# gabrielfnayres/new-vit

Hardware: AMD Instinct MI355X
Metric: volumes_per_sec_mst_dinov2_fwd (higher is better)
Workload: dtype bf16; 1 GPU; MST-DINOv2 (DinoV2ClassifierSlice, ViT-S/14) forward, 4 volumes/GPU of 64x512x512 bf16 zero-padded to 518x518 (N=1370 tokens/slice); global_batch_volumes=4, slices=64, parallelism=single GPU, weights=synthetic (mst.synth seed 2), random init of the reference architecture

## Files before the change

### new-vit_amd/csrc/k_attn16.hip

```cpp
#include <type_traits>

#include "mst_common.h"

namespace {

constexpr float LOG2E = 1.4426950408889634f;
constexpr int KV_TILE_BYTES = 64 * 128;
constexpr int K_ROW = 144, K_TILE_BYTES = 64 * K_ROW;

template <typename T>
__device__ __forceinline__ typename V8<T>::type tr_pair(const char* p_lo, const char* p_hi) {
    typedef typename V8<T>::type vec8;
    union { struct { s16x4 lo, hi; } s; vec8 v; } u;
    u.s.lo = __builtin_amdgcn_ds_read_tr16_b64_v4i16((__attribute__((address_space(3))) s16x4*)(p_lo));
    u.s.hi = __builtin_amdgcn_ds_read_tr16_b64_v4i16((__attribute__((address_space(3))) s16x4*)(p_hi));
    return u.v;
}

constexpr int ATTN_WG_WAVES = 4;
constexpr int WGW = ATTN_WG_WAVES, WGT = 64 * WGW, QB = 32 * WGW;
constexpr int ATTN_WAVES_PER_EU = 4;
template <typename T>
__global__ __launch_bounds__(WGT) __attribute__((amdgpu_waves_per_eu(ATTN_WAVES_PER_EU, ATTN_WAVES_PER_EU))) void attn16_kernel(const T* __restrict__ qkv, T* __restrict__ out,
                                                     int N, int heads, int log2q, int out_blocked) {
    typedef typename V8<T>::type vec8;
    __shared__ __attribute__((aligned(16))) char smem[4 * KV_TILE_BYTES];
    char* const Ks = smem;
    char* const Vs = smem + 2 * KV_TILE_BYTES;

    const int tid = threadIdx.x, lane = tid & 63;
    const int wave = __builtin_amdgcn_readfirstlane(tid >> 6);
    const int nqb = (N + QB - 1) / QB;
    const int tile = xcd_remap(blockIdx.x, gridDim.x);
    const int qb = tile % nqb, h = (tile / nqb) % heads, seq = tile / (nqb * heads);
    const int E = heads * 64, ld = 3 * E;
    const T* base = qkv + (int64_t)seq * N * ld;
    const int h2 = lane >> 5;

    const int q = qb * QB + wave * 32 + (lane & 31);
    const bool wave_active = (qb * QB + wave * 32) < N;
    vec8 bq[4];
    {
        const int qc = q < N ? q : N - 1;
        const T* qp = base + (int64_t)qc * ld + h * 64 + h2 * 8;
#pragma unroll
        for (int ds = 0; ds < 4; ++ds) bq[ds] = *reinterpret_cast<const vec8*>(qp + ds * 16);
    }

    static_assert(WGW == 4 || WGW == 8, "the LDS-DMA staging map deals 16 pieces per tile to 4 or 8 waves");
    constexpr int PPW = 16 / WGW;
    const int d_p0 = wave * PPW;
    const int d_row0 = (d_p0 & 7) * 8 + (lane >> 3);
    const int d_isv = d_p0 >> 3;
    const int d_chunk0 = d_isv ? ((lane & 7) ^ (((d_row0 >> 1) & 1) << 2)) : ((lane & 7) ^ ((d_row0 >> 1) & 7));
    const int d_col0 = (1 + d_isv) * (heads * 64) + h * 64 + d_chunk0 * 8;
    unsigned d_off[PPW];
#pragma unroll
    for (int u = 0; u < PPW; ++u) d_off[u] = (unsigned)(((d_row0 + 8 * u) * ld + ((u & 1) && !d_isv ? (d_col0 ^ 32) : d_col0)) * 2);
    auto dma = [&](int t, int buf) {
        char* dst = (d_isv ? Vs + buf * KV_TILE_BYTES : Ks + buf * KV_TILE_BYTES) + (d_p0 & 7) * 1024;
        if (t * 64 + 64 <= N) {
            const char* tb = reinterpret_cast<const char*>(base) + (int64_t)t * 64 * ld * 2;
#pragma unroll
            for (int u = 0; u < PPW; ++u) {
                const unsigned m0v = (unsigned)(size_t)(__attribute__((address_space(3))) char*)(dst + u * 1024);
#pragma clang diagnostic push
#pragma clang diagnostic ignored "-Winline-asm"
                asm volatile("s_mov_b32 m0, %2\n\ts_nop 0\n\tglobal_load_lds_dwordx4 %0, %1"
                             :
                             : "v"(d_off[u]), "s"(tb), "s"(m0v)
                             : "memory", "m0");
#pragma clang diagnostic pop
            }
        } else {
#pragma unroll
            for (int u = 0; u < PPW; ++u) {
                int key = t * 64 + d_row0 + 8 * u;
                key = key < N ? key : N - 1;
                const int col = (u & 1) && !d_isv ? (d_col0 ^ 32) : d_col0;
                __builtin_amdgcn_global_load_lds(GLB_PTR(base + (int64_t)key * ld + col), LDS_PTR(dst + u * 1024), 16, 0, 0);
            }
        }
    };
    const int krow = lane & 31;
    int k_off4[4];
#pragma unroll
    for (int ds = 0; ds < 4; ++ds) k_off4[ds] = krow * 128 + (((2 * ds + h2) ^ ((krow >> 1) & 7)) << 4);
    const int vi = lane & 15;
    const int vrow = 4 * h2 + (vi >> 2);
    const int vsw = ((vrow >> 1) & 1) << 2;
    const int vchunk = ((lane >> 4) & 1) * 2 + ((vi & 3) >> 1);
    const int v_lane_off = vrow * 128 + (vi & 1) * 8;

    f32x16 oT[2];
#pragma unroll
    for (int r = 0; r < 16; ++r) oT[0][r] = oT[1][r] = 0.f;
    if (!log2q) {
#pragma unroll
        for (int ds = 0; ds < 4; ++ds)
#pragma unroll
            for (int j = 0; j < 8; ++j) bq[ds][j] = (T)((float)bq[ds][j] * LOG2E);
    }
    float r_ref = 0.f, l_run = 0.f;
    constexpr float RT = 8.0f;

    const int nt = (N + 63) >> 6;
    dma(0, 0);
    asm volatile("s_waitcnt vmcnt(0)" ::: "memory");
    __syncthreads();

    constexpr float TH0 = std::is_same<T, f16_t>::value ? 8.0f : 60.0f;
    constexpr float GUARD = std::is_same<T, f16_t>::value ? 32768.0f : 1.2676506e30f;
    bool fast = false;

    auto tile_step = [&](auto mask_tag, auto fast_tag, int t, bool skip_dma) -> bool {
        constexpr bool MASK = decltype(mask_tag)::value;
        constexpr bool FAST = decltype(fast_tag)::value;
        const int buf = t & 1;
        if (t + 1 < nt && !skip_dma) dma(t + 1, buf ^ 1);
        if (wave_active) {
            const char* Kb = Ks + buf * KV_TILE_BYTES;
            const char* Vb = Vs + buf * KV_TILE_BYTES;
            f32x16 s[2];
            const f32x16 zero16 = {0.f, 0.f, 0.f, 0.f, 0.f, 0.f, 0.f, 0.f, 0.f, 0.f, 0.f, 0.f, 0.f, 0.f, 0.f, 0.f};
            const bool upper = !MASK || (t * 64 + 32 < N);
            auto scores = [&](bool with_ref) {
                vec8 kone, qneg;
                if (with_ref) {
#pragma unroll
                    for (int j = 0; j < 8; ++j) kone[j] = qneg[j] = (T)0.f;
                    if (h2 == 0) {
                        kone[0] = (T)1.f;
                        qneg[0] = (T)(-r_ref);
                    }
                }
#pragma unroll
                for (int kb = 0; kb < 2; ++kb) {
                    if (MASK && kb == 1 && !upper) {
#pragma unroll
                        for (int r = 0; r < 16; ++r) s[1][r] = -INFINITY;
                        continue;
                    }
                    s[kb] = with_ref ? mfma32(kone, qneg, zero16) : zero16;
#pragma unroll
                    for (int ds = 0; ds < 4; ++ds) {
                        const vec8 a = *reinterpret_cast<const vec8*>(Kb + k_off4[ds] + kb * 4096);
                        s[kb] = mfma32(a, bq[ds], s[kb]);
                    }
                }
                if constexpr (MASK) {
#pragma unroll
                    for (int kb = 0; kb < 2; ++kb)
#pragma unroll
                        for (int r = 0; r < 16; ++r) {
                            const int key = t * 64 + kb * 32 + (r & 3) + 8 * (r >> 2) + 4 * h2;
                            if (key >= N) s[kb][r] = -INFINITY;
                        }
                }
            };
            float lsum;
            vec8 pf[4];
            auto exps = [&]() {
                lsum = 0.f;
#pragma unroll
                for (int kb = 0; kb < 2; ++kb)
#pragma unroll
                    for (int r = 0; r < 16; ++r) {
                        const float p = __builtin_amdgcn_exp2f(s[kb][r]);
                        s[kb][r] = p;
                        lsum += p;
                    }
#pragma unroll
                for (int ks = 0; ks < 4; ++ks)
#pragma unroll
                    for (int j = 0; j < 8; ++j) pf[ks][j] = (T)s[ks >> 1][(ks & 1) * 8 + j];
            };
            auto classic = [&]() {
                float mx = s[0][0];
#pragma unroll
                for (int r = 1; r < 16; ++r) mx = fmaxf(mx, s[0][r]);
#pragma unroll
                for (int r = 0; r < 16; ++r) mx = fmaxf(mx, s[1][r]);
                {
                    const unsigned mu = __float_as_uint(mx);
                    const auto sw = __builtin_amdgcn_permlane32_swap(mu, mu, false, false);
                    mx = fmaxf(__uint_as_float(sw[0]), __uint_as_float(sw[1]));
                }
                if (t == 0 && __all(fabsf(mx) <= TH0)) {
                    fast = true;
                } else if (t == 0 || !__all(mx <= RT)) {
                    const bool mv = (t == 0) || (mx > RT);
                    const float r_new = mv ? (float)(T)(r_ref + mx) : r_ref;
                    const float delta = r_new - r_ref;
                    const float alpha = t == 0 ? 1.0f : __builtin_amdgcn_exp2f(-delta);
                    r_ref = r_new;
                    l_run *= alpha;
#pragma unroll
                    for (int r = 0; r < 16; ++r) {
                        oT[0][r] *= alpha;
                        oT[1][r] *= alpha;
                        s[0][r] -= delta;
                        s[1][r] -= delta;
                    }
                }
                exps();
            };
            if constexpr (FAST) {
                scores(false);
                exps();
                if (!__all(lsum < GUARD)) return false;
            } else {
                scores(true);
                classic();
            }
            l_run += lsum;
#pragma unroll
            for (int ks = 0; ks < 4; ++ks) {
                if (MASK && ks >= 2 && !upper) continue;
#pragma unroll
                for (int db = 0; db < 2; ++db) {
                    const char* p = Vb + ks * 16 * 128 + v_lane_off + (((db * 4 + vchunk) ^ vsw) * 16);
                    const vec8 vf = tr_pair<T>(p, p + 8 * 128);
                    oT[db] = mfma32(vf, pf[ks], oT[db]);
                }
            }
        }
        asm volatile("s_waitcnt vmcnt(0)" ::: "memory");
        __syncthreads();
        return true;
    };
    const int nt_full = (N & 63) ? nt - 1 : nt;
    const std::false_type FULL{}, CLASSIC{};
    const std::true_type RAGGED{}, FASTM{};
    if (nt_full > 0) tile_step(FULL, CLASSIC, 0, false);
    else tile_step(RAGGED, CLASSIC, 0, false);
    int t = 1;
    bool resume = false;
    if (fast) {
        for (; t < nt_full; ++t)
            if (!tile_step(FULL, FASTM, t, false)) { resume = true; break; }
    }
    for (; t < nt_full; ++t) {
        tile_step(FULL, CLASSIC, t, resume);
        resume = false;
    }
    if (t < nt) tile_step(RAGGED, CLASSIC, t, resume);

    if (wave_active) {
        const float l_tot = l_run + __shfl_xor(l_run, 32, 64);
        const float inv = 1.0f / l_tot;
        if (q < N) {
            const int64_t R = (int64_t)seq * N + q;
            T* op = out_blocked ? out + (R >> 5) * (32 * E) + (4 * h) * 512 + (R & 31) * 8 + 4 * h2
                                : out + R * E + h * 64 + 4 * h2;
            const int sdb = out_blocked ? 1024 : 32, sg2 = out_blocked ? 512 : 16, sg1 = out_blocked ? 256 : 8;
#pragma unroll
            for (int db = 0; db < 2; ++db)
#pragma unroll
                for (int g = 0; g < 4; ++g) {
                    typedef __attribute__((ext_vector_type(4))) T o4;
                    o4 pk;
#pragma unroll
                    for (int e = 0; e < 4; ++e) pk[e] = (T)(oT[db][g * 4 + e] * inv);
                    *reinterpret_cast<o4*>(op + db * sdb + (g >> 1) * sg2 + (g & 1) * sg1) = pk;
                }
        }
    }
}

template <typename T>
__global__ __launch_bounds__(256) void cls_probs_kernel(const T* __restrict__ qkv, float* __restrict__ probs,
                                                        int N, int heads, int hd, int log2q, T* __restrict__ attn_out = nullptr) {
    extern __shared__ float sm[];
    float* q0 = sm;
    float* sc = sm + hd;
    float* red = sc + N;
    const int h = blockIdx.x, seq = blockIdx.y, tid = threadIdx.x;
    const int E = heads * hd, ld = 3 * E;
    const T* base = qkv + (int64_t)seq * N * ld;
    for (int d = tid; d < hd; d += 256) q0[d] = to_f32(base[h * hd + d]);
    __syncthreads();
    float mx = -INFINITY;
    if (hd == 64) {
        const int sub = tid & 7;
        float qr[8];
#pragma unroll
        for (int i = 0; i < 8; ++i) qr[i] = q0[sub * 8 + i];
        for (int j0 = 0; j0 < N; j0 += 32) {
            const int j = j0 + (tid >> 3);
            const T* kp = base + (int64_t)(j < N ? j : N - 1) * ld + E + h * 64 + sub * 8;
            float a = 0.f;
#pragma unroll
            for (int i = 0; i < 8; ++i) a = fmaf(qr[i], to_f32(kp[i]), a);
            a += __shfl_xor(a, 1, 64);
            a += __shfl_xor(a, 2, 64);
            a += __shfl_xor(a, 4, 64);
            if (j < N) {
                if (sub == 0) sc[j] = a;
                mx = fmaxf(mx, a);
            }
        }
    } else {
        for (int j = tid; j < N; j += 256) {
            const T* kp = base + (int64_t)j * ld + E + h * hd;
            float a = 0.f;
            for (int d = 0; d < hd; ++d) a = fmaf(q0[d], to_f32(kp[d]), a);
            sc[j] = a;
            mx = fmaxf(mx, a);
        }
    }
    mx = wave_max(mx);
    if ((tid & 63) == 0) red[tid >> 6] = mx;
    __syncthreads();
    mx = fmaxf(fmaxf(red[0], red[1]), fmaxf(red[2], red[3]));
    float sum = 0.f;
    for (int j = tid; j < N; j += 256) {
        const float p = log2q ? exp2f(sc[j] - mx) : __expf(sc[j] - mx);
        sc[j] = p;
        sum += p;
    }
    sum = wave_sum(sum);
    if ((tid & 63) == 0) red[4 + (tid >> 6)] = sum;
    __syncthreads();
    const float inv = 1.0f / (red[4] + red[5] + red[6] + red[7]);
    if (probs) {
        float* po = probs + ((int64_t)seq * heads + h) * N;
        for (int j = tid; j < N; j += 256) po[j] = sc[j] * inv;
    }
    if (attn_out) {
        float* part = red + 8;
        const int d = tid & 63, pt = tid >> 6;
        const int per = (N + 3) >> 2;
        const int j1 = (pt + 1) * per < N ? (pt + 1) * per : N;
        float a = 0.f;
        for (int j = pt * per; j < j1; ++j) a = fmaf(sc[j], to_f32(base[(int64_t)j * ld + 2 * E + h * 64 + d]), a);
        part[pt * 64 + d] = a;
        __syncthreads();
        if (tid < 64) attn_out[(int64_t)seq * E + h * 64 + tid] = (T)(((part[tid] + part[64 + tid]) + (part[128 + tid] + part[192 + tid])) * inv);
    }
}

template <typename T>
__global__ __launch_bounds__(256) void probs_full_kernel(const T* __restrict__ qkv, float* __restrict__ probs,
                                                         int N, int heads, int hd, int log2q) {
    extern __shared__ float sm[];
    const int lane = threadIdx.x & 63, wave = threadIdx.x >> 6;
    float* qv = sm + wave * (hd + N);
    float* sc = qv + hd;
    const int h = blockIdx.y, seq = blockIdx.z;
    const int qi = blockIdx.x * 4 + wave;
    if (qi >= N) return;
    const int E = heads * hd, ld = 3 * E;
    const T* base = qkv + (int64_t)seq * N * ld;
    for (int d = lane; d < hd; d += 64) qv[d] = to_f32(base[(int64_t)qi * ld + h * hd + d]);
    __builtin_amdgcn_wave_barrier();
    float mx = -INFINITY;
    for (int j = lane; j < N; j += 64) {
        const T* kp = base + (int64_t)j * ld + E + h * hd;
        float a = 0.f;
        for (int d = 0; d < hd; ++d) a = fmaf(qv[d], to_f32(kp[d]), a);
        sc[j] = a;
        mx = fmaxf(mx, a);
    }
    mx = wave_max(mx);
    float sum = 0.f;
    for (int j = lane; j < N; j += 64) {
        const float p = log2q ? exp2f(sc[j] - mx) : __expf(sc[j] - mx);
        sc[j] = p;
        sum += p;
    }
    const float inv = 1.0f / wave_sum(sum);
    float* po = probs + (((int64_t)seq * heads + h) * N + qi) * N;
    for (int j = lane; j < N; j += 64) po[j] = sc[j] * inv;
}

template <typename T>
__global__ __launch_bounds__(256) void probs_full16_kernel(const T* __restrict__ qkv, float* __restrict__ probs, int N,
                                                           int heads, int log2q) {
    typedef typename V8<T>::type vec8;
    __shared__ __attribute__((aligned(16))) char smem[2 * K_TILE_BYTES + 128 * 8];
    char* const Ks = smem;
    float* const stat = reinterpret_cast<float*>(smem + 2 * K_TILE_BYTES);
    const int tid = threadIdx.x, lane = tid & 63;
    const int wave = __builtin_amdgcn_readfirstlane(tid >> 6);
    const int nqb = (N + 127) >> 7;
    const int tile = xcd_remap(blockIdx.x, gridDim.x);
    const int qb = tile % nqb, h = (tile / nqb) % heads, seq = tile / (nqb * heads);
    const int E = heads * 64, ld = 3 * E;
    const T* base = qkv + (int64_t)seq * N * ld;
    const int h2 = lane >> 5;
    const int q = qb * 128 + wave * 32 + (lane & 31);
    const float sc = log2q ? 1.0f : LOG2E;
    vec8 bq[4];
    {
        const int qc = q < N ? q : N - 1;
        const T* qp = base + (int64_t)qc * ld + h * 64 + h2 * 8;
#pragma unroll
        for (int ds = 0; ds < 4; ++ds) bq[ds] = *reinterpret_cast<const vec8*>(qp + ds * 16);
    }
    const int sr = tid >> 2, sc0 = (tid & 3) * 2;
    u32x4 rk0, rk1;
    auto gload = [&](int t) {
        int key = t * 64 + sr;
        key = key < N ? key : N - 1;
        const T* kp = base + (int64_t)key * ld + E + h * 64 + sc0 * 8;
        rk0 = *reinterpret_cast<const u32x4*>(kp);
        rk1 = *reinterpret_cast<const u32x4*>(kp + 8);
    };
    auto lstore = [&](int buf) {
        *reinterpret_cast<u32x4*>(Ks + buf * K_TILE_BYTES + sr * K_ROW + sc0 * 16) = rk0;
        *reinterpret_cast<u32x4*>(Ks + buf * K_TILE_BYTES + sr * K_ROW + sc0 * 16 + 16) = rk1;
    };
    const int k_lane_off = (lane & 31) * K_ROW + h2 * 16;
    const int nt = (N + 63) >> 6;
    const f32x16 zero16 = {0.f, 0.f, 0.f, 0.f, 0.f, 0.f, 0.f, 0.f, 0.f, 0.f, 0.f, 0.f, 0.f, 0.f, 0.f, 0.f};

    float m_run = -INFINITY, l_run = 0.f;
    gload(0);
    lstore(0);
    __syncthreads();
    for (int t = 0; t < nt; ++t) {
        const int buf = t & 1;
        if (t + 1 < nt) gload(t + 1);
        const char* Kb = Ks + buf * K_TILE_BYTES;
        f32x16 s[2];
#pragma unroll
        for (int kb = 0; kb < 2; ++kb) {
            s[kb] = zero16;
#pragma unroll
            for (int ds = 0; ds < 4; ++ds) {
                const vec8 a = *reinterpret_cast<const vec8*>(Kb + k_lane_off + kb * 32 * K_ROW + ds * 32);
                s[kb] = mfma32(a, bq[ds], s[kb]);
            }
        }
        float mx = -INFINITY;
#pragma unroll
        for (int kb = 0; kb < 2; ++kb)
#pragma unroll
            for (int r = 0; r < 16; ++r) {
                const int key = t * 64 + kb * 32 + (r & 3) + 8 * (r >> 2) + 4 * h2;
                s[kb][r] = key < N ? s[kb][r] * sc : -INFINITY;
                mx = fmaxf(mx, s[kb][r]);
            }
        mx = fmaxf(mx, __shfl_xor(mx, 32, 64));
        const float m_new = fmaxf(m_run, mx);
        float lsum = 0.f;
#pragma unroll
        for (int kb = 0; kb < 2; ++kb)
#pragma unroll
            for (int r = 0; r < 16; ++r) lsum += __builtin_amdgcn_exp2f(s[kb][r] - m_new);
        l_run = l_run * __builtin_amdgcn_exp2f(m_run - m_new) + lsum;
        m_run = m_new;
        if (t + 1 < nt) lstore(buf ^ 1);
        __syncthreads();
    }
    {
        const float l_tot = l_run + __shfl_xor(l_run, 32, 64);
        if (h2 == 0) {
            stat[(wave * 32 + (lane & 31)) * 2] = m_run;
            stat[(wave * 32 + (lane & 31)) * 2 + 1] = 1.0f / l_tot;
        }
    }
    __syncthreads();

    float mrow[16], irow[16];
#pragma unroll
    for (int r = 0; r < 16; ++r) {
        const int ql = wave * 32 + (r & 3) + 8 * (r >> 2) + 4 * h2;
        mrow[r] = stat[ql * 2];
        irow[r] = stat[ql * 2 + 1];
    }
    float* const pbase = probs + (((int64_t)seq * heads + h) * N) * N;
    gload(0);
    __syncthreads();
    lstore(0);
    __syncthreads();
    for (int t = 0; t < nt; ++t) {
        const int buf = t & 1;
        if (t + 1 < nt) gload(t + 1);
        const char* Kb = Ks + buf * K_TILE_BYTES;
#pragma unroll
        for (int kb = 0; kb < 2; ++kb) {
            f32x16 s = zero16;
#pragma unroll
            for (int ds = 0; ds < 4; ++ds) {
                const vec8 a = *reinterpret_cast<const vec8*>(Kb + k_lane_off + kb * 32 * K_ROW + ds * 32);
                s = mfma32(bq[ds], a, s);
            }
            const int key = t * 64 + kb * 32 + (lane & 31);
#pragma unroll
            for (int r = 0; r < 16; ++r) {
                const int qq = qb * 128 + wave * 32 + (r & 3) + 8 * (r >> 2) + 4 * h2;
                if (key < N && qq < N) pbase[(int64_t)qq * N + key] = __builtin_amdgcn_exp2f(s[r] * sc - mrow[r]) * irow[r];
            }
        }
        if (t + 1 < nt) lstore(buf ^ 1);
        __syncthreads();
    }
}

}

int launch_attn16(const void* qkv, int dt, int n_seq, int N, int heads, void* out, int log2q, hipStream_t s, int out_blocked) {
    MST_CHECK_ARG(n_seq > 0 && N > 0 && heads > 0, "attention: bad sizes n_seq=%d N=%d heads=%d", n_seq, N, heads);
    const int64_t nwg = (int64_t)((N + QB - 1) / QB) * heads * n_seq;
    MST_CHECK_ARG(nwg < (1ll << 31), "attention: grid too large");
    const dim3 grid((unsigned)nwg), block(WGT);
    if (dt == MST_BF16) attn16_kernel<bf16_t><<<grid, block, 0, s>>>((const bf16_t*)qkv, (bf16_t*)out, N, heads, log2q, out_blocked);
    else if (dt == MST_F16) attn16_kernel<f16_t><<<grid, block, 0, s>>>((const f16_t*)qkv, (f16_t*)out, N, heads, log2q, out_blocked);
    else { mst_set_error("attention16: bad dtype %d", dt); return MST_EINVAL; }
    return mst_check_launch("attention16");
}

int launch_cls_probs(const void* qkv, int dt, int n_seq, int N, int heads, int hd, float* probs, int log2q, hipStream_t s) {
    MST_CHECK_ARG(N > 0 && N <= 12000 && hd > 0 && hd <= 256, "cls_probs: N=%d hd=%d unsupported", N, hd);
    if (n_seq > 65535) {
        const size_t esz = dt == MST_F32 ? 4 : 2;
        for (int s0 = 0; s0 < n_seq; s0 += 65535) {
            const int c = (n_seq - s0 < 65535) ? n_seq - s0 : 65535;
            int rc = launch_cls_probs((const char*)qkv + (size_t)s0 * N * 3 * heads * hd * esz, dt, c, N, heads, hd,
                                      probs + (size_t)s0 * heads * N, log2q, s);
            if (rc) return rc;
        }
        return MST_OK;
    }
    const dim3 grid(heads, n_seq), block(256);
    const size_t sh = (size_t)(hd + N + 8 + 256) * sizeof(float);
    if (dt == MST_BF16) cls_probs_kernel<bf16_t><<<grid, block, sh, s>>>((const bf16_t*)qkv, probs, N, heads, hd, log2q);
    else if (dt == MST_F16) cls_probs_kernel<f16_t><<<grid, block, sh, s>>>((const f16_t*)qkv, probs, N, heads, hd, log2q);
    else if (dt == MST_F32) cls_probs_kernel<float><<<grid, block, sh, s>>>((const float*)qkv, probs, N, heads, hd, log2q);
    else { mst_set_error("cls_probs: bad dtype %d", dt); return MST_EINVAL; }
    return mst_check_launch("cls_probs");
}

int launch_cls_attn(const void* qkv, int dt, int n_seq, int N, int heads, float* probs, void* out, int log2q, hipStream_t s) {
    MST_CHECK_ARG(N > 0 && N <= 12000 && n_seq > 0 && n_seq <= 65535 && out, "cls_attn: N=%d n_seq=%d unsupported", N, n_seq);
    const dim3 grid(heads, n_seq), block(256);
    const size_t sh = (size_t)(64 + N + 8 + 256) * sizeof(float);
    if (dt == MST_BF16) cls_probs_kernel<bf16_t><<<grid, block, sh, s>>>((const bf16_t*)qkv, probs, N, heads, 64, log2q, (bf16_t*)out);
    else if (dt == MST_F16) cls_probs_kernel<f16_t><<<grid, block, sh, s>>>((const f16_t*)qkv, probs, N, heads, 64, log2q, (f16_t*)out);
    else if (dt == MST_F32) cls_probs_kernel<float><<<grid, block, sh, s>>>((const float*)qkv, probs, N, heads, 64, log2q, (float*)out);
    else { mst_set_error("cls_attn: bad dtype %d", dt); return MST_EINVAL; }
    return mst_check_launch("cls_attn");
}

int launch_probs_full(const void* qkv, int dt, int n_seq, int N, int heads, int hd, float* probs, int log2q, hipStream_t s) {
    if (hd == 64 && (dt == MST_BF16 || dt == MST_F16)) {
        MST_CHECK_ARG(N > 0 && n_seq > 0 && heads > 0, "probs_full: bad sizes");
        const int64_t nwg = (int64_t)((N + 127) / 128) * heads * n_seq;
        MST_CHECK_ARG(nwg < (1ll << 31), "probs_full: grid too large");
        if (dt == MST_BF16) probs_full16_kernel<bf16_t><<<dim3((unsigned)nwg), dim3(256), 0, s>>>((const bf16_t*)qkv, probs, N, heads, log2q);
        else probs_full16_kernel<f16_t><<<dim3((unsigned)nwg), dim3(256), 0, s>>>((const f16_t*)qkv, probs, N, heads, log2q);
        return mst_check_launch("probs_full16");
    }
    MST_CHECK_ARG(N > 0 && N <= 3800 && hd > 0 && hd <= 256, "probs_full: N=%d hd=%d unsupported", N, hd);
    if (n_seq > 65535) {
        const size_t esz = dt == MST_F32 ? 4 : 2;
        for (int s0 = 0; s0 < n_seq; s0 += 65535) {
            const int c = (n_seq - s0 < 65535) ? n_seq - s0 : 65535;
            int rc = launch_probs_full((const char*)qkv + (size_t)s0 * N * 3 * heads * hd * esz, dt, c, N, heads, hd,
                                       probs + (size_t)s0 * heads * N * N, log2q, s);
            if (rc) return rc;
        }
        return MST_OK;
    }
    const dim3 grid((N + 3) / 4, heads, n_seq), block(256);
    const size_t sh = (size_t)4 * (hd + N) * sizeof(float);
    if (dt == MST_BF16) probs_full_kernel<bf16_t><<<grid, block, sh, s>>>((const bf16_t*)qkv, probs, N, heads, hd, log2q);
    else if (dt == MST_F16) probs_full_kernel<f16_t><<<grid, block, sh, s>>>((const f16_t*)qkv, probs, N, heads, hd, log2q);
    else if (dt == MST_F32) probs_full_kernel<float><<<grid, block, sh, s>>>((const float*)qkv, probs, N, heads, hd, log2q);
    else { mst_set_error("probs_full: bad dtype %d", dt); return MST_EINVAL; }
    return mst_check_launch("probs_full");
}
```

Before: 166.6 volumes/s.

## Process two query groups per wave in attention to reuse K/V fragments

The attention kernel is templated on G query groups per wave. With G=2 each wave handles 64 queries, so every K and V LDS fragment read feeds two MFMAs. Full 256-row query blocks go to the G=2 variant, which runs at 2 waves/EU, and the remainder rows go to a second G=1 launch. This cuts LDS reads and KV tile staging per query, at the cost of more registers, lower occupancy, an extra kernel launch, and per-group fast-path tracking.

```diff
diff --git a/new-vit_amd/csrc/k_attn16.hip b/new-vit_amd/csrc/k_attn16.hip
--- a/new-vit_amd/csrc/k_attn16.hip
+++ b/new-vit_amd/csrc/k_attn16.hip
@@ -18,11 +18,11 @@
 }
 
 constexpr int ATTN_WG_WAVES = 4;
-constexpr int WGW = ATTN_WG_WAVES, WGT = 64 * WGW, QB = 32 * WGW;
-constexpr int ATTN_WAVES_PER_EU = 4;
-template <typename T>
-__global__ __launch_bounds__(WGT) __attribute__((amdgpu_waves_per_eu(ATTN_WAVES_PER_EU, ATTN_WAVES_PER_EU))) void attn16_kernel(const T* __restrict__ qkv, T* __restrict__ out,
-                                                     int N, int heads, int log2q, int out_blocked) {
+constexpr int WGW = ATTN_WG_WAVES, WGT = 64 * WGW;
+template <typename T, int G>
+__global__ __launch_bounds__(WGT) __attribute__((amdgpu_waves_per_eu(G == 1 ? 4 : 2, G == 1 ? 4 : 2))) void attn16_kernel(const T* __restrict__ qkv, T* __restrict__ out,
+                                                     int N, int heads, int log2q, int out_blocked, int q_begin, int q_end) {
+    constexpr int QB = 32 * G * WGW;
     typedef typename V8<T>::type vec8;
     __shared__ __attribute__((aligned(16))) char smem[4 * KV_TILE_BYTES];
     char* const Ks = smem;
@@ -30,21 +30,22 @@
 
     const int tid = threadIdx.x, lane = tid & 63;
     const int wave = __builtin_amdgcn_readfirstlane(tid >> 6);
-    const int nqb = (N + QB - 1) / QB;
+    const int nqb = (q_end - q_begin + QB - 1) / QB;
     const int tile = xcd_remap(blockIdx.x, gridDim.x);
     const int qb = tile % nqb, h = (tile / nqb) % heads, seq = tile / (nqb * heads);
     const int E = heads * 64, ld = 3 * E;
     const T* base = qkv + (int64_t)seq * N * ld;
     const int h2 = lane >> 5;
 
-    const int q = qb * QB + wave * 32 + (lane & 31);
-    const bool wave_active = (qb * QB + wave * 32) < N;
-    vec8 bq[4];
-    {
-        const int qc = q < N ? q : N - 1;
+    const int q0 = q_begin + qb * QB + wave * (32 * G) + (lane & 31);
+    const bool wave_active = (q_begin + qb * QB + wave * (32 * G)) < N;
+    vec8 bq[G][4];
+#pragma unroll
+    for (int g = 0; g < G; ++g) {
+        const int qc = q0 + 32 * g < N ? q0 + 32 * g : N - 1;
         const T* qp = base + (int64_t)qc * ld + h * 64 + h2 * 8;
 #pragma unroll
-        for (int ds = 0; ds < 4; ++ds) bq[ds] = *reinterpret_cast<const vec8*>(qp + ds * 16);
+        for (int ds = 0; ds < 4; ++ds) bq[g][ds] = *reinterpret_cast<const vec8*>(qp + ds * 16);
     }
 
     static_assert(WGW == 4 || WGW == 8, "the LDS-DMA staging map deals 16 pieces per tile to 4 or 8 waves");
@@ -92,16 +93,22 @@
     const int vchunk = ((lane >> 4) & 1) * 2 + ((vi & 3) >> 1);
     const int v_lane_off = vrow * 128 + (vi & 1) * 8;
 
-    f32x16 oT[2];
-#pragma unroll
-    for (int r = 0; r < 16; ++r) oT[0][r] = oT[1][r] = 0.f;
+    f32x16 oT[G][2];
+#pragma unroll
+    for (int g = 0; g < G; ++g)
+#pragma unroll
+        for (int r = 0; r < 16; ++r) oT[g][0][r] = oT[g][1][r] = 0.f;
     if (!log2q) {
 #pragma unroll
-        for (int ds = 0; ds < 4; ++ds)
-#pragma unroll
-            for (int j = 0; j < 8; ++j) bq[ds][j] = (T)((float)bq[ds][j] * LOG2E);
-    }
-    float r_ref = 0.f, l_run = 0.f;
+        for (int g = 0; g < G; ++g)
+#pragma unroll
+            for (int ds = 0; ds < 4; ++ds)
+#pragma unroll
+                for (int j = 0; j < 8; ++j) bq[g][ds][j] = (T)((float)bq[g][ds][j] * LOG2E);
+    }
+    float r_ref[G], l_run[G];
+#pragma unroll
+    for (int g = 0; g < G; ++g) r_ref[g] = l_run[g] = 0.f;
     constexpr float RT = 8.0f;
 
     const int nt = (N + 63) >> 6;
@@ -111,7 +118,9 @@
 
     constexpr float TH0 = std::is_same<T, f16_t>::value ? 8.0f : 60.0f;
     constexpr float GUARD = std::is_same<T, f16_t>::value ? 32768.0f : 1.2676506e30f;
-    bool fast = false;
+    bool fast[G];
+#pragma unroll
+    for (int g = 0; g < G; ++g) fast[g] = false;
 
     auto tile_step = [&](auto mask_tag, auto fast_tag, int t, bool skip_dma) -> bool {
         constexpr bool MASK = decltype(mask_tag)::value;
@@ -121,31 +130,38 @@
         if (wave_active) {
             const char* Kb = Ks + buf * KV_TILE_BYTES;
             const char* Vb = Vs + buf * KV_TILE_BYTES;
-            f32x16 s[2];
+            f32x16 s[G][2];
             const f32x16 zero16 = {0.f, 0.f, 0.f, 0.f, 0.f, 0.f, 0.f, 0.f, 0.f, 0.f, 0.f, 0.f, 0.f, 0.f, 0.f, 0.f};
             const bool upper = !MASK || (t * 64 + 32 < N);
             auto scores = [&](bool with_ref) {
-                vec8 kone, qneg;
+                vec8 kone, qneg[G];
                 if (with_ref) {
 #pragma unroll
-                    for (int j = 0; j < 8; ++j) kone[j] = qneg[j] = (T)0.f;
-                    if (h2 == 0) {
-                        kone[0] = (T)1.f;
-                        qneg[0] = (T)(-r_ref);
+                    for (int j = 0; j < 8; ++j) kone[j] = (T)0.f;
+                    if (h2 == 0) kone[0] = (T)1.f;
+#pragma unroll
+                    for (int g = 0; g < G; ++g) {
+#pragma unroll
+                        for (int j = 0; j < 8; ++j) qneg[g][j] = (T)0.f;
+                        if (h2 == 0) qneg[g][0] = (T)(-r_ref[g]);
                     }
                 }
 #pragma unroll
                 for (int kb = 0; kb < 2; ++kb) {
                     if (MASK && kb == 1 && !upper) {
 #pragma unroll
-                        for (int r = 0; r < 16; ++r) s[1][r] = -INFINITY;
+                        for (int g = 0; g < G; ++g)
+#pragma unroll
+                            for (int r = 0; r < 16; ++r) s[g][1][r] = -INFINITY;
                         continue;
                     }
-                    s[kb] = with_ref ? mfma32(kone, qneg, zero16) : zero16;
+#pragma unroll
+                    for (int g = 0; g < G; ++g) s[g][kb] = with_ref ? mfma32(kone, qneg[g], zero16) : zero16;
 #pragma unroll
                     for (int ds = 0; ds < 4; ++ds) {
                         const vec8 a = *reinterpret_cast<const vec8*>(Kb + k_off4[ds] + kb * 4096);
-                        s[kb] = mfma32(a, bq[ds], s[kb]);
+#pragma unroll
+                        for (int g = 0; g < G; ++g) s[g][kb] = mfma32(a, bq[g][ds], s[g][kb]);
                     }
                 }
                 if constexpr (MASK) {
@@ -154,53 +170,70 @@
 #pragma unroll
                         for (int r = 0; r < 16; ++r) {
                             const int key = t * 64 + kb * 32 + (r & 3) + 8 * (r >> 2) + 4 * h2;
-                            if (key >= N) s[kb][r] = -INFINITY;
+#pragma unroll
+                            for (int g = 0; g < G; ++g)
+                                if (key >= N) s[g][kb][r] = -INFINITY;
                         }
                 }
             };
-            float lsum;
-            vec8 pf[4];
+            float lsum[G];
+            vec8 pf[G][4];
             auto exps = [&]() {
-                lsum = 0.f;
-#pragma unroll
-                for (int kb = 0; kb < 2; ++kb)
-#pragma unroll
-                    for (int r = 0; r < 16; ++r) {
-                        const float p = __builtin_amdgcn_exp2f(s[kb][r]);
-                        s[kb][r] = p;
-                        lsum += p;
-                    }
-#pragma unroll
-                for (int ks = 0; ks < 4; ++ks)
-#pragma unroll
-                    for (int j = 0; j < 8; ++j) pf[ks][j] = (T)s[ks >> 1][(ks & 1) * 8 + j];
+#pragma unroll
+                for (int g = 0; g < G; ++g) {
+                    lsum[g] = 0.f;
+#pragma unroll
+                    for (int kb = 0; kb < 2; ++kb)
+#pragma unroll
+                        for (int r = 0; r < 16; ++r) {
+                            const float p = __builtin_amdgcn_exp2f(s[g][kb][r]);
+                            s[g][kb][r] = p;
+                            lsum[g] += p;
+                        }
+#pragma unroll
+                    for (int ks = 0; ks < 4; ++ks)
+#pragma unroll
+                        for (int j = 0; j < 8; ++j) pf[g][ks][j] = (T)s[g][ks >> 1][(ks & 1) * 8 + j];
+                }
             };
             auto classic = [&]() {
-                float mx = s[0][0];
-#pragma unroll
-                for (int r = 1; r < 16; ++r) mx = fmaxf(mx, s[0][r]);
-#pragma unroll
-                for (int r = 0; r < 16; ++r) mx = fmaxf(mx, s[1][r]);
-                {
-                    const unsigned mu = __float_as_uint(mx);
-                    const auto sw = __builtin_amdgcn_permlane32_swap(mu, mu, false, false);
-                    mx = fmaxf(__uint_as_float(sw[0]), __uint_as_float(sw[1]));
-                }
-                if (t == 0 && __all(fabsf(mx) <= TH0)) {
-                    fast = true;
-                } else if (t == 0 || !__all(mx <= RT)) {
-                    const bool mv = (t == 0) || (mx > RT);
-                    const float r_new = mv ? (float)(T)(r_ref + mx) : r_ref;
-                    const float delta = r_new - r_ref;
-                    const float alpha = t == 0 ? 1.0f : __builtin_amdgcn_exp2f(-delta);
-                    r_ref = r_new;
-                    l_run *= alpha;
-#pragma unroll
-                    for (int r = 0; r < 16; ++r) {
-                        oT[0][r] *= alpha;
-                        oT[1][r] *= alpha;
-                        s[0][r] -= delta;
-                        s[1][r] -= delta;
+#pragma unroll
+                for (int g = 0; g < G; ++g) {
+                    if (!MASK && fast[g]) {
+                        float tsum = 0.f;
+#pragma unroll
+                        for (int kb = 0; kb < 2; ++kb)
+#pragma unroll
+                            for (int r = 0; r < 16; ++r) tsum += __builtin_amdgcn_exp2f(s[g][kb][r]);
+                        if (__all(tsum < GUARD)) continue;
+                        fast[g] = false;
+                    }
+                    float m = s[g][0][0];
+#pragma unroll
+                    for (int r = 1; r < 16; ++r) m = fmaxf(m, s[g][0][r]);
+#pragma unroll
+                    for (int r = 0; r < 16; ++r) m = fmaxf(m, s[g][1][r]);
+                    {
+                        const unsigned mu = __float_as_uint(m);
+                        const auto sw = __builtin_amdgcn_permlane32_swap(mu, mu, false, false);
+                        m = fmaxf(__uint_as_float(sw[0]), __uint_as_float(sw[1]));
+                    }
+                    if (t == 0 && __all(fabsf(m) <= TH0)) {
+                        fast[g] = true;
+                    } else if (t == 0 || !__all(m <= RT)) {
+                        const bool mv = (t == 0) || (m > RT);
+                        const float r_new = mv ? (float)(T)(r_ref[g] + m) : r_ref[g];
+                        const float delta = r_new - r_ref[g];
+                        const float alpha = t == 0 ? 1.0f : __builtin_amdgcn_exp2f(-delta);
+                        r_ref[g] = r_new;
+                        l_run[g] *= alpha;
+#pragma unroll
+                        for (int r = 0; r < 16; ++r) {
+                            oT[g][0][r] *= alpha;
+                            oT[g][1][r] *= alpha;
+                            s[g][0][r] -= delta;
+                            s[g][1][r] -= delta;
+                        }
                     }
                 }
                 exps();
@@ -208,12 +241,16 @@
             if constexpr (FAST) {
                 scores(false);
                 exps();
-                if (!__all(lsum < GUARD)) return false;
+                bool in_range = true;
+#pragma unroll
+                for (int g = 0; g < G; ++g) in_range = in_range && (lsum[g] < GUARD);
+                if (!__all(in_range)) return false;
             } else {
                 scores(true);
                 classic();
             }
-            l_run += lsum;
+#pragma unroll
+            for (int g = 0; g < G; ++g) l_run[g] += lsum[g];
 #pragma unroll
             for (int ks = 0; ks < 4; ++ks) {
                 if (MASK && ks >= 2 && !upper) continue;
@@ -221,7 +258,8 @@
                 for (int db = 0; db < 2; ++db) {
                     const char* p = Vb + ks * 16 * 128 + v_lane_off + (((db * 4 + vchunk) ^ vsw) * 16);
                     const vec8 vf = tr_pair<T>(p, p + 8 * 128);
-                    oT[db] = mfma32(vf, pf[ks], oT[db]);
+#pragma unroll
+                    for (int g = 0; g < G; ++g) oT[g][db] = mfma32(vf, pf[g][ks], oT[g][db]);
                 }
             }
         }
@@ -236,7 +274,10 @@
     else tile_step(RAGGED, CLASSIC, 0, false);
     int t = 1;
     bool resume = false;
-    if (fast) {
+    bool all_fast = true;
+#pragma unroll
+    for (int g = 0; g < G; ++g) all_fast = all_fast && fast[g];
+    if (all_fast) {
         for (; t < nt_full; ++t)
             if (!tile_step(FULL, FASTM, t, false)) { resume = true; break; }
     }
@@ -247,7 +288,10 @@
     if (t < nt) tile_step(RAGGED, CLASSIC, t, resume);
 
     if (wave_active) {
-        const float l_tot = l_run + __shfl_xor(l_run, 32, 64);
+#pragma unroll
+      for (int g = 0; g < G; ++g) {
+        const int q = q0 + 32 * g;
+        const float l_tot = l_run[g] + __shfl_xor(l_run[g], 32, 64);
         const float inv = 1.0f / l_tot;
         if (q < N) {
             const int64_t R = (int64_t)seq * N + q;
@@ -257,14 +301,15 @@
 #pragma unroll
             for (int db = 0; db < 2; ++db)
 #pragma unroll
-                for (int g = 0; g < 4; ++g) {
+                for (int c = 0; c < 4; ++c) {
                     typedef __attribute__((ext_vector_type(4))) T o4;
                     o4 pk;
 #pragma unroll
-                    for (int e = 0; e < 4; ++e) pk[e] = (T)(oT[db][g * 4 + e] * inv);
-                    *reinterpret_cast<o4*>(op + db * sdb + (g >> 1) * sg2 + (g & 1) * sg1) = pk;
+                    for (int e = 0; e < 4; ++e) pk[e] = (T)(oT[g][db][c * 4 + e] * inv);
+                    *reinterpret_cast<o4*>(op + db * sdb + (c >> 1) * sg2 + (c & 1) * sg1) = pk;
                 }
         }
+      }
     }
 }
 
@@ -499,16 +544,30 @@
     }
 }
 
+bool attn16_wide_applicable(int n_seq, int N, int heads) {
+    return N >= 64 * WGW;
+}
+
 }
 
 int launch_attn16(const void* qkv, int dt, int n_seq, int N, int heads, void* out, int log2q, hipStream_t s, int out_blocked) {
     MST_CHECK_ARG(n_seq > 0 && N > 0 && heads > 0, "attention: bad sizes n_seq=%d N=%d heads=%d", n_seq, N, heads);
-    const int64_t nwg = (int64_t)((N + QB - 1) / QB) * heads * n_seq;
-    MST_CHECK_ARG(nwg < (1ll << 31), "attention: grid too large");
-    const dim3 grid((unsigned)nwg), block(WGT);
-    if (dt == MST_BF16) attn16_kernel<bf16_t><<<grid, block, 0, s>>>((const bf16_t*)qkv, (bf16_t*)out, N, heads, log2q, out_blocked);
-    else if (dt == MST_F16) attn16_kernel<f16_t><<<grid, block, 0, s>>>((const f16_t*)qkv, (f16_t*)out, N, heads, log2q, out_blocked);
-    else { mst_set_error("attention16: bad dtype %d", dt); return MST_EINVAL; }
+    MST_CHECK_ARG(dt == MST_BF16 || dt == MST_F16, "attention16: bad dtype %d", dt);
+    const int wide_rows = attn16_wide_applicable(n_seq, N, heads) ? (N / (64 * WGW)) * (64 * WGW) : 0;
+    const int64_t nwg2 = (int64_t)(wide_rows / (64 * WGW)) * heads * n_seq;
+    const int64_t nwg1 = (int64_t)((N - wide_rows + 32 * WGW - 1) / (32 * WGW)) * heads * n_seq;
+    MST_CHECK_ARG(nwg1 < (1ll << 31) && nwg2 < (1ll << 31), "attention: grid too large");
+    const dim3 block(WGT);
+    if (nwg2) {
+        const dim3 grid((unsigned)nwg2);
+        if (dt == MST_BF16) attn16_kernel<bf16_t, 2><<<grid, block, 0, s>>>((const bf16_t*)qkv, (bf16_t*)out, N, heads, log2q, out_blocked, 0, wide_rows);
+        else attn16_kernel<f16_t, 2><<<grid, block, 0, s>>>((const f16_t*)qkv, (f16_t*)out, N, heads, log2q, out_blocked, 0, wide_rows);
+    }
+    if (nwg1) {
+        const dim3 grid((unsigned)nwg1);
+        if (dt == MST_BF16) attn16_kernel<bf16_t, 1><<<grid, block, 0, s>>>((const bf16_t*)qkv, (bf16_t*)out, N, heads, log2q, out_blocked, wide_rows, N);
+        else attn16_kernel<f16_t, 1><<<grid, block, 0, s>>>((const f16_t*)qkv, (f16_t*)out, N, heads, log2q, out_blocked, wide_rows, N);
+    }
     return mst_check_launch("attention16");
 }
 
```

New measurement: 162.0 volumes/s. -2.8%, worse.
